# dylanhogan/aggfly

Hardware: AMD Instinct MI355X
Metric: grid-cell-timesteps/s (fused transform+weighted reduce) (higher is better)
Workload: dtype f64

## Files before the change

### aggfly_amd/csrc/afhip_api.hip

```cpp
#include <hip/hip_runtime.h>

#include <algorithm>
#include <cmath>
#include <cstdio>
#include <cstdlib>
#include <cstring>
#include <mutex>
#include <string>
#include <vector>

#include "../../include/aggfly_hip.h"
#include "afhip_kernels.h"
#include "afhip_panel_kernels.h"
#include "afhip_lz4_kernels.h"
#include "afhip_zstd_kernels.h"
#include "afhip_inflate_kernels.h"
#include "afhip_planner.h"
#include "afhip_variants.h"
#include "afhip_sine_p2_table.h"

using namespace afhip;

namespace {

// ... 887 lines not shown
        fa.hb_shift = pl->wg == 64 ? 6 : (pl->wg == 128 ? 7 : 8);
        for (int i = 0; i < MAX_THR; ++i) fa.hb_bin_of_slot[i] = pl->hb_bin_of_slot[i];
        for (int k = 0; k <= pl->hb_n; ++k) {
            const double t = pl->hb_edge[k];
            const float f = (float)t;
            fa.hb_edge[k] = t;
            fa.hb_dn[k] = (double)f > t ? std::nextafterf(f, -INFINITY) : f;
            fa.hb_up[k] = (double)f < t ? std::nextafterf(f, INFINITY) : f;
        }
        fa.hb_w = pl->hb_w; fa.hb_lo0 = pl->hb_lo0; fa.hb_gl = pl->hb_gl; fa.hb_gh = pl->hb_gh;
        fa.hb_wf = (float)pl->hb_w; fa.hb_lo0f = (float)pl->hb_lo0; fa.hb_glf = (float)pl->hb_gl; fa.hb_ghf = (float)pl->hb_gh;
        fa.hb_c0b = pl->hb_c0b; fa.hb_c0bf = (float)pl->hb_c0b;
    }
    HIP_TRY(hipLaunchKernel(fn, grid, dim3((unsigned)pl->wg), args, lds, st));
    return AFHIP_OK;
}

static int launch_combine(afhip_plan* pl, const double* partial, double* cells, double* panel, hipStream_t st) {
    const int64_t C = pl->desc.n_cells, P = pl->desc.P;
    if (P == 0) return AFHIP_OK;
    CombineArgs ca{};
    ca.partial = partial; ca.slot_ptr = pl->d_slot_ptr.p; ca.outer_bounds = pl->d_ob.p;
    ca.cells_out = cells; ca.panel = panel; ca.C = C; ca.P = P; ca.K = pl->K;
    ca.pk = pl->packed ? pl->pk : PackFmt{};
    for (int j = 0; j < pl->K; ++j) {
        ca.outer[j] = pl->cols[(size_t)j].outer;
        ca.round_final[j] = (pl->cols[(size_t)j].rounding & AFHIP_ROUND_FINAL) ? 1 : 0;
    }
    if (P >= 4 && panel) {
        dim3 grid((unsigned)((C + CT_CELLS - 1) / CT_CELLS), (unsigned)((P + CT_PER - 1) / CT_PER));
        if (grid.y > 65535) return fail(AFHIP_E_UNSUPPORTED, "more than 524,280 output periods in one call");
        hipLaunchKernelGGL(k_combine_slots_tiled, grid, dim3(WG), 0, st, ca);
    } else {
        dim3 grid((unsigned)((C + WG - 1) / WG), (unsigned)std::min<int64_t>(P, 65535));
        hipLaunchKernelGGL(k_combine_slots, grid, dim3(WG), 0, st, ca);
    }
    HIP_TRY(hipGetLastError());
    return AFHIP_OK;
}

static int launch_spmm_slots(afhip_plan* pl, const afhip_csr* csr, const double* partial, hipStream_t st,
                             double* num_dev, double* den_dev, double* res_dev, bool* divided) {
    const int64_t P = pl->desc.P, K = pl->K, Q = (K + 1) * P;
    if (csr->nseg * P == 0) return AFHIP_OK;
    SlotSpmmArgs sa{};
    sa.seg_ptr = csr->seg_ptr.p; sa.dst = csr->seg_dst.p; sa.cols = csr->cols.p; sa.w = csr->w.p;
    sa.partial = partial; sa.slot_ptr = pl->d_slot_ptr.p; sa.outer_bounds = pl->d_ob.p; sa.out = pl->sums;
    sa.nseg = csr->nseg; sa.P = P; sa.C = pl->desc.n_cells; sa.K = (int32_t)K;
    sa.p_major = pl->slot_spmm_order >= 0 ? pl->slot_spmm_order : (P >= 8 ? 1 : 0);
    *divided = csr->n_split == 0 && csr->nseg == csr->R;
    if (*divided) { sa.num = num_dev; sa.den = den_dev; sa.res = res_dev; sa.R = csr->R; }
    for (int j = 0; j < pl->K; ++j) {
        sa.outer[j] = pl->cols[(size_t)j].outer;
        sa.round_final[j] = (pl->cols[(size_t)j].rounding & AFHIP_ROUND_FINAL) ? 1 : 0;
    }
    const int64_t mean_len = csr->nnz / std::max<int64_t>(csr->nseg, 1);
    int sub = mean_len > 32 ? 64 : (mean_len > 16 ? 32 : (mean_len > 8 ? 16 : 8));
    if (pl->slot_spmm_sub) sub = pl->slot_spmm_sub;
    const int64_t pairs = csr->nseg * P;
    const int64_t blocks = (pairs * sub + WG - 1) / WG;
    if (blocks > INT32_MAX) return fail(AFHIP_E_UNSUPPORTED, "plan_run: %lld (segment, period) pairs in one call", (long long)pairs);
#define AFHIP_SLOTS_SUB(KB)                                                                                                   \
    switch (sub) {                                                                                                            \
        case 8: hipLaunchKernelGGL((k_csr_spmm_slots<KB, 8>), dim3((unsigned)blocks), dim3(WG), 0, st, sa); break;            \
        case 16: hipLaunchKernelGGL((k_csr_spmm_slots<KB, 16>), dim3((unsigned)blocks), dim3(WG), 0, st, sa); break;          \
        case 32: hipLaunchKernelGGL((k_csr_spmm_slots<KB, 32>), dim3((unsigned)blocks), dim3(WG), 0, st, sa); break;          \
        default: hipLaunchKernelGGL((k_csr_spmm_slots<KB, 64>), dim3((unsigned)blocks), dim3(WG), 0, st, sa); break;          \
    }
    if (K <= 2) { AFHIP_SLOTS_SUB(2) }
    else if (K <= 4) { AFHIP_SLOTS_SUB(4) }
    else if (K <= 8) { AFHIP_SLOTS_SUB(8) }
    else { AFHIP_SLOTS_SUB(16) }
#undef AFHIP_SLOTS_SUB
    HIP_TRY(hipGetLastError());
    if (csr->n_split) {
        const int64_t n = csr->n_split * Q;
        hipLaunchKernelGGL(k_csr_combine_segments, dim3((unsigned)((n + WG - 1) / WG)), dim3(WG), 0, st, pl->sums, csr->split_row.p,
                           csr->split_ptr.p, csr->R, Q, csr->n_split);
        HIP_TRY(hipGetLastError());
    }
    return AFHIP_OK;
}

static int ensure_ws(afhip_plan* pl, int64_t bytes, void* user_ws, int64_t user_bytes, const char* who, char** base) {
    if (user_ws) {
        if (user_bytes < bytes)
            return fail(AFHIP_E_INVALID, "%s: the workspace holds %lld bytes, the run needs %lld (afhip_plan_run_workspace_bytes / afhip_plan_workspace_bytes)",
                        who, (long long)user_bytes, (long long)bytes);
        if ((uintptr_t)user_ws % 256 != 0) return fail(AFHIP_E_INVALID, "%s: the workspace must be 256-byte aligned", who);
        int rc = check_ptr_device(pl, user_ws, who, "the workspace");
        if (rc) return rc;
        *base = (char*)user_ws;
        pl->last_ws = 1;
        return AFHIP_OK;
    }
    if (pl->own_ws_bytes < bytes) {
        if (pl->own_ws) { pl->retired.push_back(pl->own_ws); pl->own_ws = nullptr; pl->own_ws_bytes = 0; }
        HIP_TRY(hipMalloc(&pl->own_ws, (size_t)bytes));
        pl->own_ws_bytes = bytes;
    }
    *base = (char*)pl->own_ws;
    pl->last_ws = 2;
    return AFHIP_OK;
}

extern "C" int afhip_plan_run_temporal(afhip_plan* plan, const void* cube_dev, double* cells_dev,
                                       void* workspace_dev, int64_t workspace_bytes, void* stream) {
    if (!plan || !cube_dev || !cells_dev) return fail(AFHIP_E_INVALID, "plan_run_temporal: NULL argument");
    int rcd = check_cube_device(plan, cube_dev, "plan_run_temporal");
    if (!rcd) rcd = check_ptr_device(plan, cells_dev, "plan_run_temporal", "the per-cell output");
    if (rcd) return rcd;
    GUARD_DEVICE(plan->device);
    hipStream_t st = (hipStream_t)stream;
    char* base;
    int rc = ensure_ws(plan, plan->ws_partial, workspace_dev, workspace_bytes, "plan_run_temporal", &base);
    if (rc) return rc;
    double* partial = (double*)base;
    if ((rc = launch_temporal(plan, cube_dev, partial, st))) return rc;
    return launch_combine(plan, partial, cells_dev, nullptr, st);
}

extern "C" int afhip_plan_run(afhip_plan* plan, const void* cube_dev, const afhip_csr* csr,
                              double* num_dev, double* den_dev, double* res_dev, double* cells_dev,
                              void* workspace_dev, int64_t workspace_bytes, void* stream, float* kernel_ms) {
    if (!plan || !cube_dev || !csr || !res_dev) return fail(AFHIP_E_INVALID, "plan_run: NULL argument");
    if (csr->n_cells != plan->desc.n_cells)
        return fail(AFHIP_E_INVALID, "plan_run: CSR has %lld cells, plan has %lld", (long long)csr->n_cells, (long long)plan->desc.n_cells);
    if (csr->device != plan->device)
        return fail(AFHIP_E_INVALID, "plan_run: the CSR lives on device %d, the plan on device %d", csr->device, plan->device);
    int rcd = check_cube_device(plan, cube_dev, "plan_run");
    if (!rcd) rcd = check_ptr_device(plan, res_dev, "plan_run", "the result panel");
    if (!rcd && num_dev) rcd = check_ptr_device(plan, num_dev, "plan_run", "the numerator panel");
    if (!rcd && den_dev) rcd = check_ptr_device(plan, den_dev, "plan_run", "the denominator panel");
    if (!rcd && cells_dev) rcd = check_ptr_device(plan, cells_dev, "plan_run", "the per-cell output");
    if (rcd) return rcd;
    GUARD_DEVICE(plan->device);
    hipStream_t st = (hipStream_t)stream;
    const int64_t K = plan->K, P = plan->desc.P, Q = (K + 1) * P;
    char* base;
    int rc = ensure_ws(plan, afhip_plan_run_workspace_bytes(plan, csr), workspace_dev, workspace_bytes, "plan_run", &base);
    if (rc) return rc;
    double* partial = (double*)base;
    double* panel = (double*)(base + plan->ws_partial);
    plan->sums = (double*)(base + plan->ws_partial + plan->ws_panel);
    if (kernel_ms) {
        for (auto& e : plan->ev) if (!e) HIP_TRY(hipEventCreate(&e));
        HIP_TRY(hipEventRecord(plan->ev[0], st));
    }
    const bool exact = plan->desc.exact_order != 0 || spmm_serial_env();
    const afhip_csr::RfTab* rf = nullptr;
    if (plan->rf_plan_ok && !exact && !cells_dev && !plan->packed) {
        rf = rf_table(const_cast<afhip_csr*>(csr), plan->variant->vec);
        if (rf && plan->n_slots * (rf->n_runs + rf->n_xcells) * (K + 1) * 8 > plan->ws_partial) rf = nullptr;
    }
    const bool prof = !plan->prof_ev.empty() && (size_t)(2 * plan->prof_count + 1) < plan->prof_ev.size();
    if (prof) HIP_TRY(hipEventRecord(plan->prof_ev[(size_t)(2 * plan->prof_count)], st));
    if ((rc = launch_temporal(plan, cube_dev, partial, st, rf))) return rc;
    if (prof) { HIP_TRY(hipEventRecord(plan->prof_ev[(size_t)(2 * plan->prof_count + 1)], st)); ++plan->prof_count; }
    if (kernel_ms) HIP_TRY(hipEventRecord(plan->ev[1], st));
    plan->last_route = rf ? 1 : 0;
    plan->last_counts_lanes = -1;
    bool divided = false;
    if (rf) {
        const int64_t n = csr->R * P * (K + 1);
        if (n) {
            uint32_t mean_mask = 0;
            for (int j = 0; j < plan->K; ++j) if (plan->cols[(size_t)j].outer == OUT_MEAN) mean_mask |= 1u << j;
            hipLaunchKernelGGL(k_rf_reduce, dim3((unsigned)((n + WG - 1) / WG)), dim3(WG), 0, st, (const double*)partial, rf->reg_ptr.p, rf->reg_runs.p,
                               plan->d_slot_ptr.p, plan->d_ob.p, mean_mask, (const double*)(partial + plan->n_slots * rf->n_runs * (K + 1)), rf->n_xcells,
                               rf->xreg_ptr.p, rf->xcell.p, rf->xw.p, plan->sums, csr->R, P, (int)(K + 1), rf->n_runs,
                               rf_run_major(plan, rf) ? (int64_t)(K + 1) : rf->n_runs * (K + 1), rf_run_major(plan, rf) ? plan->n_slots * (K + 1) : (int64_t)(K + 1),
                               (!rf_run_major(plan, rf) && P >= 8) ? 1 : 0);
            HIP_TRY(hipGetLastError());
        }
    } else if (plan->packed && !cells_dev && plan->n_slots <= P && plan->counts_spmm) {
        const int64_t nv = exact ? csr->R : csr->nseg, nq = nv * P;
        if (nq) {
            divided = (exact || csr->n_split == 0) && nv == csr->R;
            const int64_t nnz_rows = csr->h_indptr.empty() ? 0 : csr->h_indptr.back();
            const double entries = nv > 0 ? (double)nnz_rows / (double)nv : 0.0;
            const int sub_rule = ((double)P < entries) ? (entries < 12.0 ? 8 : 16) : 0;
            const int sub = exact ? 0 : (plan->counts_spmm_sub >= 0 ? plan->counts_spmm_sub : sub_rule);
            plan->last_counts_lanes = (sub == 4 || sub == 8 || sub == 16) ? sub : 1;
            const int64_t* ip = exact ? csr->indptr.p : csr->seg_ptr.p;
            const int32_t* dr = exact ? (const int32_t*)nullptr : csr->seg_dst.p;
            double* o_num = divided ? num_dev : (double*)nullptr; double* o_den = divided ? den_dev : (double*)nullptr; double* o_res = divided ? res_dev : (double*)nullptr;
            if (sub == 4 || sub == 8 || sub == 16) {
                const dim3 gr((unsigned)((nq * sub + WG - 1) / WG)), bl(WG);
                if (sub == 4) hipLaunchKernelGGL((k_csr_spmm_counts_sub<4>), gr, bl, 0, st, ip, dr, csr->cols.p, csr->w.p, (const void*)partial, plan->d_slot_ptr.p, plan->sums, nv, P, (int)K, plan->desc.n_cells, plan->pk, o_num, o_den, o_res);
                else if (sub == 8) hipLaunchKernelGGL((k_csr_spmm_counts_sub<8>), gr, bl, 0, st, ip, dr, csr->cols.p, csr->w.p, (const void*)partial, plan->d_slot_ptr.p, plan->sums, nv, P, (int)K, plan->desc.n_cells, plan->pk, o_num, o_den, o_res);
                else hipLaunchKernelGGL((k_csr_spmm_counts_sub<16>), gr, bl, 0, st, ip, dr, csr->cols.p, csr->w.p, (const void*)partial, plan->d_slot_ptr.p, plan->sums, nv, P, (int)K, plan->desc.n_cells, plan->pk, o_num, o_den, o_res);
            } else
            hipLaunchKernelGGL(k_csr_spmm_counts, dim3((unsigned)((nq + WG - 1) / WG)), dim3(WG), 0, st, ip, dr, csr->cols.p,
                               csr->w.p, (const void*)partial, plan->d_slot_ptr.p, plan->sums, nv, P, (int)K, plan->desc.n_cells, plan->pk,
                               o_num, o_den, o_res);
            HIP_TRY(hipGetLastError());
            if (!exact && csr->n_split) {
                const int64_t n = csr->n_split * Q;
                hipLaunchKernelGGL(k_csr_combine_segments, dim3((unsigned)((n + WG - 1) / WG)), dim3(WG), 0, st, plan->sums, csr->split_row.p,
                                   csr->split_ptr.p, csr->R, Q, csr->n_split);
                HIP_TRY(hipGetLastError());
            }
        }
    } else if (!exact && !cells_dev && !plan->packed && K > 0 && !plan->no_slot_spmm) {
        if ((rc = launch_spmm_slots(plan, csr, partial, st, num_dev, den_dev, res_dev, &divided))) return rc;
    } else {
        if ((rc = launch_combine(plan, partial, cells_dev, panel, st))) return rc;
        if ((rc = launch_spmm(csr, panel, plan->sums, Q, st, exact))) return rc;
    }
    const int64_t n = K > 0 ? csr->R * P : 0;
    if (n && !divided) {
        hipLaunchKernelGGL(k_panel_divide, dim3((unsigned)((n + WG - 1) / WG)), dim3(WG), 0, st, plan->sums, num_dev,
                           den_dev, res_dev, csr->R, P, (int)K);
        HIP_TRY(hipGetLastError());
    }
    if (kernel_ms) {
        HIP_TRY(hipEventRecord(plan->ev[2], st));
        HIP_TRY(hipEventSynchronize(plan->ev[2]));
        HIP_TRY(hipEventElapsedTime(&kernel_ms[0], plan->ev[0], plan->ev[1]));
        HIP_TRY(hipEventElapsedTime(&kernel_ms[1], plan->ev[0], plan->ev[2]));
    }
    return AFHIP_OK;
}

extern "C" int afhip_plan_profile_begin(afhip_plan* plan, int64_t max_launches) {
    if (!plan || max_launches < 0) return fail(AFHIP_E_INVALID, "plan_profile_begin: bad arguments");
    GUARD_DEVICE(plan->device);
    for (auto& e : plan->prof_ev) if (e) (void)hipEventDestroy(e);
    plan->prof_ev.assign((size_t)(2 * max_launches), nullptr);
    for (auto& e : plan->prof_ev) HIP_TRY(hipEventCreate(&e));
    plan->prof_count = 0;
    return AFHIP_OK;
}

extern "C" int64_t afhip_plan_profile_end(afhip_plan* plan, float* ms_out, int64_t cap) {
    if (!plan) return 0;
    DeviceGuard guard__(plan->device);
    const int64_t n = plan->prof_count;
    for (int64_t i = 0; i < n && i < cap; ++i) {
        if (hipEventSynchronize(plan->prof_ev[(size_t)(2 * i + 1)]) != hipSuccess ||
            hipEventElapsedTime(&ms_out[i], plan->prof_ev[(size_t)(2 * i)], plan->prof_ev[(size_t)(2 * i + 1)]) != hipSuccess) {
            fail(AFHIP_E_HIP, "plan_profile_end: event query failed");
            return -1;
        }
    }
    for (auto& e : plan->prof_ev) if (e) (void)hipEventDestroy(e);
    plan->prof_ev.clear();
    plan->prof_count = 0;
    return n;
}

static int run_group(const void* cube_dev, int dtype, int64_t T, int64_t n_cells, const int64_t* bounds,
                     int64_t G, int code, const double* ddargs, int64_t D, void* out_dev, void* stream) {
    if (!cube_dev || !bounds || !out_dev) return fail(AFHIP_E_INVALID, "group kernel: NULL argument");
    if (G < 0 || D <= 0) return fail(AFHIP_E_INVALID, "group kernel: bad G/D");
    if (dtype != AFHIP_F32 && dtype != AFHIP_F64) return fail(AFHIP_E_INVALID, "group kernel: dtype must be AFHIP_F32 or AFHIP_F64");
    if (G == 0) return AFHIP_OK;
// ... 59 lines not shown
```

### aggfly_amd/csrc/afhip_panel_kernels.h

```cpp
#pragma once
#include "afhip_kernels.h"

namespace afhip {

struct CombineArgs {
    const double* partial;
    const int32_t* slot_ptr;
    const int64_t* outer_bounds;
    double* cells_out;
    double* panel;
    int64_t C, P;
    int32_t K;
    int32_t outer[MAX_COLS];
    int32_t round_final[MAX_COLS];
    PackFmt pk;
};

__device__ __forceinline__ double ld_partial(const double* partial, const PackFmt& pk, int64_t s, int j, int K, int64_t C, int64_t c) {
    if (pk.nw) {
        const uint64_t q = ((const uint64_t*)partial)[(s * C + c) * pk.nw + pk.word[j]];
        const uint32_t u = (uint32_t)(q >> pk.shift[j]) & pk.mask;
        return u == pk.mask ? nan64() : (double)u;
    }
    return partial[(s * K + j) * C + c];
// ... 400 lines not shown
                if (a.outer[k] == OUT_MEAN) x[k] = x[k] / ng;
                if (a.round_final[k]) x[k] = (double)(float)x[k];
                valid = valid && (x[k] == x[k]);
            }
        }
#pragma unroll
        for (int k = 0; k < KB; ++k)
            if (k < K) acc[k] = __dadd_rn(acc[k], __dmul_rn(wj, valid ? x[k] : 0.0));
        acc[KB] = __dadd_rn(acc[KB], __dmul_rn(wj, valid ? 1.0 : 0.0));
    };
    auto merged = [&](int k, int64_t c) -> double {
        double val = a.partial[((int64_t)s0 * K + k) * C + c];
        const int o = a.outer[k];
        for (int s = s0 + 1; s < s1; ++s) {
            const double x = a.partial[((int64_t)s * K + k) * C + c];
            if (o == OUT_MIN) { double t = (x < val) ? x : val; val = (x != x || val != val) ? nan64() : t; }
            else if (o == OUT_MAX) { double t = (x > val) ? x : val; val = (x != x || val != val) ? nan64() : t; }
            else if (o == OUT_FIRST) {  }
            else val += x;
        }
        return val;
    };
    if (s1 != s0) {
        const int64_t j0 = a.seg_ptr[v], j1 = a.seg_ptr[v + 1];
        int64_t j = j0 + sl;
        if (s1 == s0 + 1) {
            const double* base = a.partial + (int64_t)s0 * K * C;
            for (; j + (UNR - 1) * SUB < j1; j += UNR * SUB) {
                double x[UNR][KB], wj[UNR];
#pragma unroll
                for (int u = 0; u < UNR; ++u) {
                    const int64_t c = a.cols[j + u * SUB];
                    wj[u] = a.w[j + u * SUB];
#pragma unroll
                    for (int k = 0; k < KB; ++k) x[u][k] = (k < K) ? base[(int64_t)k * C + c] : 0.0;
                }
#pragma unroll
                for (int u = 0; u < UNR; ++u) finish(x[u], wj[u]);
            }
            for (; j < j1; j += SUB) {
                double x[KB];
                const int64_t c = a.cols[j];
#pragma unroll
                for (int k = 0; k < KB; ++k) x[k] = (k < K) ? base[(int64_t)k * C + c] : 0.0;
                finish(x, a.w[j]);
            }
        } else {
            for (; j < j1; j += SUB) {
                double x[KB];
                const int64_t c = a.cols[j];
#pragma unroll
                for (int k = 0; k < KB; ++k) x[k] = (k < K) ? merged(k, c) : 0.0;
                finish(x, a.w[j]);
            }
        }
    }
#pragma unroll
    for (int m = SUB / 2; m >= 1; m >>= 1) {
#pragma unroll
        for (int k = 0; k <= KB; ++k)
            if (k < K || k == KB) acc[k] = __dadd_rn(acc[k], __shfl_xor(acc[k], m, 64));
    }
    if (sl == 0 && live) {
        if (a.res != nullptr) {
            const int64_t RP = a.R * a.P, rp = (int64_t)a.dst[v] * a.P + p;
            const double de = acc[KB];
            if (a.den) a.den[rp] = de;
#pragma unroll
            for (int k = 0; k < KB; ++k) {
                if (k >= K) continue;
                if (a.num) a.num[(int64_t)k * RP + rp] = acc[k];
                a.res[(int64_t)k * RP + rp] = (de != 0.0) ? acc[k] / de : nan64();
            }
            return;
        }
        double* o = a.out + ((int64_t)a.dst[v] * a.P + p) * (K + 1);
#pragma unroll
        for (int k = 0; k < KB; ++k)
            if (k < K) o[k] = acc[k];
        o[K] = acc[KB];
    }
}

__global__ __launch_bounds__(WG) void k_rf_reduce(const double* __restrict__ rf_out, const int64_t* __restrict__ reg_ptr,
                                                  const int32_t* __restrict__ reg_runs, const int32_t* __restrict__ slot_ptr,
                                                  const int64_t* __restrict__ outer_bounds, uint32_t mean_mask,
                                                  const double* __restrict__ ex, int64_t nx, const int64_t* __restrict__ xreg_ptr,
                                                  const int32_t* __restrict__ xcell, const double* __restrict__ xw,
                                                  double* __restrict__ sums, int64_t R, int64_t P, int K1, int64_t n_runs,
                                                  int64_t slot_stride, int64_t run_stride, int p_major) {
    const int64_t tid = (int64_t)blockIdx.x * WG + threadIdx.x;
    if (tid >= R * P * K1) return;
    const int k = (int)(tid % K1);
    const int64_t rp = tid / K1;
    const int64_t r = p_major ? rp % R : rp / P, p = p_major ? rp / R : rp - r * P;
    const int s0 = slot_ptr[p], s1 = slot_ptr[p + 1];
    double acc = 0.0;
    if (s1 != s0) {
        const double* base = rf_out + (int64_t)s0 * slot_stride + k;
        int64_t q = reg_ptr[r];
        const int64_t q1 = reg_ptr[r + 1];
        for (; q + 8 <= q1; q += 8) {
            double v[8];
#pragma unroll
            for (int u = 0; u < 8; ++u) v[u] = base[(int64_t)reg_runs[q + u] * run_stride];
#pragma unroll
            for (int u = 0; u < 8; ++u) acc = __dadd_rn(acc, v[u]);
        }
        for (; q < q1; ++q) acc = __dadd_rn(acc, base[(int64_t)reg_runs[q] * run_stride]);
        if (nx) {
            const double* xb = ex + (int64_t)s0 * nx * K1 + k;
            for (int64_t x = xreg_ptr[r]; x < xreg_ptr[r + 1]; ++x) acc = __dadd_rn(acc, __dmul_rn(xw[x], xb[(int64_t)xcell[x] * K1]));
        }
        if ((mean_mask >> k) & 1u) acc = acc / (double)(outer_bounds[p + 1] - outer_bounds[p]);
    }
    sums[(r * P + p) * K1 + k] = acc;
}

__global__ __launch_bounds__(WG) void k_csr_combine_segments(double* __restrict__ sums, const int32_t* __restrict__ split_row,
                                                             const int32_t* __restrict__ split_ptr, int64_t R, int64_t Q, int64_t n_split) {
    const int64_t tid = (int64_t)blockIdx.x * WG + threadIdx.x;
    if (tid >= n_split * Q) return;
    const int64_t i = tid / Q, q = tid - i * Q;
    double a = 0.0;
    for (int64_t k = split_ptr[i]; k < split_ptr[i + 1]; ++k) a = __dadd_rn(a, sums[(R + k) * Q + q]);
    sums[(int64_t)split_row[i] * Q + q] = a;
}

__global__ __launch_bounds__(WG) void k_panel_divide(const double* __restrict__ sums, double* __restrict__ num,
                                                     double* __restrict__ den, double* __restrict__ res,
                                                     int64_t R, int64_t P, int K) {
    const int64_t rp = (int64_t)blockIdx.x * WG + threadIdx.x;
    const int64_t RP = R * P;
    if (rp >= RP) return;
    const double* rec = sums + rp * (K + 1);
    double v[MAX_COLS + 1];
#pragma unroll
    for (int k = 0; k <= MAX_COLS; ++k) v[k] = (k <= K) ? rec[k] : 0.0;
    double de = 0.0;
#pragma unroll
    for (int k = 0; k <= MAX_COLS; ++k) if (k == K) de = v[k];
    if (den) den[rp] = de;
#pragma unroll
    for (int k = 0; k < MAX_COLS; ++k) {
        if (k >= K) continue;
        if (num) num[(int64_t)k * RP + rp] = v[k];
        res[(int64_t)k * RP + rp] = (de != 0.0) ? v[k] / de : nan64();
    }
}

__global__ __launch_bounds__(WG) void k_divide_num_den(const double* __restrict__ num, const double* __restrict__ den,
                                                       double* __restrict__ res, int64_t n, int64_t RP) {
    const int64_t i = (int64_t)blockIdx.x * WG + threadIdx.x;
    if (i >= n) return;
    const double de = den[i % RP];
    res[i] = (de != 0.0) ? num[i] / de : nan64();
}

__global__ __launch_bounds__(WG) void k_validity_panel(const double* __restrict__ x, double* __restrict__ panel,
                                                       int64_t C, int64_t nt, int K) {
    const int64_t tid = (int64_t)blockIdx.x * WG + threadIdx.x;
    if (tid >= C * nt) return;
    const int64_t c = tid / nt, t = tid - c * nt;
    const int64_t Q = (int64_t)(K + 1) * nt;
    bool valid = true;
    for (int j = 0; j < K; ++j) { const double v = x[((int64_t)j * C + c) * nt + t]; valid = valid && (v == v); }
    for (int j = 0; j < K; ++j) {
        const double v = x[((int64_t)j * C + c) * nt + t];
        panel[c * Q + t * (K + 1) + j] = valid ? v : 0.0;
    }
    panel[c * Q + t * (K + 1) + K] = valid ? 1.0 : 0.0;
}

__global__ __launch_bounds__(WG) void k_unpack_i16(const int16_t* __restrict__ q, int64_t n, const PackArgs p, float* __restrict__ out) {
    const int64_t e0 = ((int64_t)blockIdx.x * WG + threadIdx.x) * 4;
    if (e0 >= n) return;
    if (e0 + 4 <= n) {
        const RawVec<int16_t, 4> r = *(const RawVec<int16_t, 4>*)(q + e0);
        float f[4];
        unpack_i16<4>(r.v, p, f);
        typedef float f4 __attribute__((ext_vector_type(4)));
        *(f4*)(out + e0) = f4{f[0], f[1], f[2], f[3]};
    } else {
        for (int64_t e = e0; e < n; ++e) {
            const int16_t one[1] = {q[e]};
            float f[1];
            unpack_i16<1>(one, p, f);
            out[e] = f[0];
        }
    }
}

constexpr int TRANSFORM_PER_THREAD = 4;
struct TransformArgs {
    const void* x;
    const void* other;
    void* out;
    int64_t n;
    int32_t x_f32, other_f32, out_f32, tf, iarg, pad;
// ... 79 lines not shown
```

### aggfly_amd/csrc/afhip_planner.cpp

```cpp
#include "afhip_planner.h"

#include <algorithm>
#include <cmath>
#include <cstdarg>
#include <cstdio>
#include <cstdlib>
#include <cstring>
#include <string>

namespace afhip {

namespace {
thread_local std::string g_err;
}

int fail(int code, const char* fmt, ...) {
    char buf[1024];
    va_list ap;
    va_start(ap, fmt);
    vsnprintf(buf, sizeof buf, fmt, ap);
    va_end(ap);
    g_err = buf;
    return code;
}

const char* last_error() { return g_err.c_str(); }

PlanKnobs read_knobs() {
    auto set = [](const char* name) { return getenv(name) != nullptr; };
    PlanKnobs k;
    if (const char* e = getenv("AFHIP_FORCE_WG")) { int w = atoi(e); if (w == 64 || w == 128 || w == 256) k.force_wg = w; }
    if (const char* e = getenv("AFHIP_WGS_PER_CU")) k.wgs_per_cu = std::max(1, atoi(e));
    k.no_period_chunks = set("AFHIP_NO_PERIOD_CHUNKS");
    k.no_round_fill = set("AFHIP_NO_ROUND_FILL");
    k.no_pair_mode = set("AFHIP_NO_PAIR_MODE");
    k.no_quad_mode = set("AFHIP_NO_QUAD_MODE");
    k.no_ragged_mode = set("AFHIP_NO_RAGGED_MODE");
    k.no_region_fused = set("AFHIP_NO_REGION_FUSED");
    k.counts_spmm = !set("AFHIP_NO_COUNTS_SPMM");
    if (const char* e = getenv("AFHIP_COUNTS_SPMM_SUB")) k.counts_spmm_sub = atoi(e);
    if (const char* e = getenv("AFHIP_NO_SLOT_SPMM")) k.no_slot_spmm = atoi(e) != 0;
    if (const char* e = getenv("AFHIP_RF_LAYOUT")) k.rf_layout = (e[0] == 'r') ? 1 : 0;
    if (const char* e = getenv("AFHIP_SLOT_SPMM_ORDER")) k.slot_spmm_order = (e[0] == 'p') ? 1 : 0;
    if (const char* e = getenv("AFHIP_SLOT_SPMM_SUB")) { const int sb = atoi(e); if (sb == 8 || sb == 16 || sb == 32 || sb == 64) k.slot_spmm_sub = sb; }
    return k;
}

static int add_thr_slot(std::vector<ThrSlot>& thr, const double* a3, bool bins) {
    ThrSlot s{};
    s.t0 = a3[0]; s.t1 = a3[1];
    const bool base_is_t0 = (a3[2] == 0.0);
    if (bins) { s.A = 0.0; s.B = 1.0; }
    else if (base_is_t0) { s.A = 1.0; s.B = -a3[0]; }
    else { s.A = -1.0; s.B = a3[1]; }
    s.t0f = (float)a3[0]; if ((double)s.t0f > a3[0]) s.t0f = std::nextafterf(s.t0f, -INFINITY);
    s.t1f = (float)a3[1]; if ((double)s.t1f < a3[1]) s.t1f = std::nextafterf(s.t1f, INFINITY);
    s.nan_poisons = bins ? 0 : 1;
    for (size_t i = 0; i < thr.size(); ++i)
        if (!memcmp(&thr[i], &s, sizeof s)) return (int)i;
    thr.push_back(s);
    return (int)thr.size() - 1;
}

static int lower_columns(PlanLayout* pl) {
    const int K = pl->desc.K;
    int stat = 0;
    pl->thr.clear(); pl->cols.clear();
    pl->has_sine = false;
    for (int j = 0; j < K; ++j) {
        const afhip_column& c = pl->columns[j];
        ColOp co{};
        co.rounding = c.rounding;
        switch (c.inner) {
            case AFHIP_MEAN: co.src = SRC_MEAN; stat = std::max(stat, 1); break;
            case AFHIP_SUM: co.src = SRC_SUM; stat = std::max(stat, 1); break;
            case AFHIP_MIN: co.src = SRC_MIN; stat = std::max(stat, 2); break;
            case AFHIP_MAX: co.src = SRC_MAX; stat = std::max(stat, 2); break;
            case AFHIP_NANMEAN: co.src = SRC_NANMEAN; stat = 3; break;
            case AFHIP_DD: co.src = SRC_THR; co.src_idx = add_thr_slot(pl->thr, c.inner_args, false); break;
            case AFHIP_BINS: co.src = SRC_THR; co.src_idx = add_thr_slot(pl->thr, c.inner_args, true); break;
            case AFHIP_SINE_DD:
                co.src = SRC_SINE; stat = std::max(stat, 2);
                co.s0 = c.inner_args[0]; co.s1 = c.inner_args[1];
                co.s0x2 = 2.0 * co.s0; co.s1x2 = 2.0 * co.s1;
                {
                    auto dn = [](double t) { float f = (float)t; return (double)f > t ? std::nextafterf(f, -INFINITY) : f; };
                    auto up = [](double t) { float f = (float)t; return (double)f < t ? std::nextafterf(f, INFINITY) : f; };
                    co.s0dn = dn(co.s0); co.s0up = up(co.s0); co.s1dn = dn(co.s1); co.s1up = up(co.s1);
                }
                co.swidth = co.s1 - co.s0; co.swidth2 = 2.0 * co.swidth;
                pl->has_sine = true;
                if (c.inner_args[2] != 0.0 && c.inner_args[2] != 1.0)
                    return fail(AFHIP_E_INVALID, "column %d: sine_dd flag must be 0 or 1 (temporal.py:324)", j);
                co.skind = (int)c.inner_args[2];
                break;
            default: return fail(AFHIP_E_INVALID, "column %d: unknown inner reducer %d", j, c.inner);
        }
        switch (c.transform) {
            case AFHIP_TF_NONE: co.tf = TF_NONE; break;
            case AFHIP_TF_POW: {
                const double e = c.transform_arg;
                if (e == std::floor(e) && std::fabs(e) <= 64.0) { co.tf = TF_POWI; co.tf_iarg = (int)e; }
                else { co.tf = TF_POW; co.tf_arg = e; }
                break;
            }
            case AFHIP_TF_HINGE: co.tf = TF_HINGE; co.tf_arg = c.transform_arg; break;
            case AFHIP_TF_INTER: co.tf = TF_INTER; break;
            default: return fail(AFHIP_E_INVALID, "column %d: unknown transform %d", j, c.transform);
        }
        if (co.tf == TF_POW || co.tf == TF_INTER) stat = 3;
        switch (c.outer) {
            case AFHIP_IDENTITY: co.outer = OUT_FIRST; break;
            case AFHIP_SUM: co.outer = OUT_SUM; break;
            case AFHIP_MEAN: co.outer = OUT_MEAN; break;
            case AFHIP_MIN: co.outer = OUT_MIN; break;
            case AFHIP_MAX: co.outer = OUT_MAX; break;
            case AFHIP_DD:
            case AFHIP_BINS:
                co.outer = c.outer == AFHIP_DD ? OUT_DD : OUT_BINS;
                co.o0 = c.outer_args[0]; co.o1 = c.outer_args[1];
                co.obase = (c.outer_args[2] == 0.0) ? c.outer_args[0] : c.outer_args[1];
                break;
            default:
                return fail(AFHIP_E_UNSUPPORTED, "column %d: outer reducer %d is not fused (use the staged path)", j, c.outer);
        }
// ... 491 lines not shown
```

### aggfly_amd/csrc/afhip_planner.h

```cpp
#pragma once
#include <stddef.h>
#include <stdint.h>

#include <vector>

#include "../../include/aggfly_hip.h"
#include "afhip_plan_types.h"
#include "afhip_variants.h"

namespace afhip {

int fail(int code, const char* fmt, ...) __attribute__((format(printf, 2, 3)));
const char* last_error();

struct DeviceFacts {
    int cu_count = 0;
    int (*resident_wgs)(const void* fn, int wg, size_t lds) = nullptr;
};

struct RunKnobs {
    bool counts_spmm = true;
    int counts_spmm_sub = -1;
    bool no_slot_spmm = false;
    int slot_spmm_sub = 0;
    int slot_spmm_order = -1;
    int rf_layout = -1;
};

struct PlanKnobs : RunKnobs {
    int force_wg = 0;
    int wgs_per_cu = 0;
    bool no_period_chunks = false, no_round_fill = false;
    bool no_pair_mode = false, no_quad_mode = false, no_ragged_mode = false;
    bool no_region_fused = false;
};
PlanKnobs read_knobs();

struct HistPartition {
    int hb_n = 0; double hb_c1 = 0, hb_c0 = 0;
    bool hb_arith = false; double hb_w = 0, hb_lo0 = 0, hb_gl = 0, hb_gh = 0, hb_c0b = 0;
    int hb_bin_of_slot[MAX_THR] = {0};
    double hb_edge[MAX_THR + 1] = {0};
};

struct PlanLayout : RunKnobs, HistPartition {
    bool has_sine = false;
    afhip_plan_desc desc{};
    std::vector<int64_t> ib, ob;
    std::vector<afhip_column> columns;
    int stat = 0, nthr = 0, K = 0;
    std::vector<ThrSlot> thr;
    std::vector<ColOp> cols;
    std::vector<ChunkDesc> chunks;
    std::vector<int32_t> emit;
    std::vector<int64_t> gtab;
    std::vector<int32_t> slot_ptr;
    int64_t n_slots = 0;
    const Variant* variant = nullptr;
    const Variant* variant_rf = nullptr;
    bool rf_plan_ok = false;
    int64_t tiles = 0;
    int wg = WG;
    bool packed = false;
    PackFmt pk{};
    int64_t ws_partial = 0, ws_panel = 0;
};

int build_plan(const afhip_plan_desc* desc, const DeviceFacts& dev, PlanLayout* out);

size_t plan_lds_bytes(const PlanLayout* pl);

}
```

Measured before the change: 862.4 billion.

## Fuse region-fused reduce with divide/finish and process all columns per thread

Replaces the per-(region,period,column) k_rf_reduce kernel with k_rf_finish, where each thread handles one (region,period) pair across all K+1 columns. Records are read with 2-wide vector loads, and numerator, denominator and ratio are written directly, so the separate divide/finish pass over the sums buffer is skipped (divided=true). An optional LDS transpose tiles regions by periods so the outputs are written in coalesced order. The trade is more registers per thread and fewer threads when R*P is small.

New measurement: 861.3 billion. Within noise of the previous version (-0.1%).

```diff
diff --git a/aggfly_amd/csrc/afhip_api.hip b/aggfly_amd/csrc/afhip_api.hip
--- a/aggfly_amd/csrc/afhip_api.hip
+++ b/aggfly_amd/csrc/afhip_api.hip
@@ -993,6 +993,43 @@
     return AFHIP_OK;
 }
 
+static int launch_rf_finish(afhip_plan* pl, const afhip_csr* csr, const afhip_csr::RfTab* rf, const double* partial, hipStream_t st,
+                            double* num_dev, double* den_dev, double* res_dev) {
+    const int64_t P = pl->desc.P, K = pl->K, R = csr->R;
+    if (K == 0 || R * P == 0) return AFHIP_OK;
+    const bool run_major = rf_run_major(pl, rf);
+    RfFinishArgs fa{};
+    fa.rf_out = partial; fa.reg_ptr = rf->reg_ptr.p; fa.reg_runs = rf->reg_runs.p;
+    fa.slot_ptr = pl->d_slot_ptr.p; fa.outer_bounds = pl->d_ob.p;
+    fa.ex = partial + pl->n_slots * rf->n_runs * (K + 1); fa.nx = rf->n_xcells;
+    fa.xreg_ptr = rf->xreg_ptr.p; fa.xcell = rf->xcell.p; fa.xw = rf->xw.p;
+    fa.num = num_dev; fa.den = den_dev; fa.res = res_dev;
+    fa.R = R; fa.P = P; fa.K = (int32_t)K;
+    fa.slot_stride = run_major ? (int64_t)(K + 1) : rf->n_runs * (K + 1);
+    fa.run_stride = run_major ? pl->n_slots * (K + 1) : (int64_t)(K + 1);
+    for (int j = 0; j < pl->K; ++j) if (pl->cols[(size_t)j].outer == OUT_MEAN) fa.mean_mask |= 1u << j;
+    int tp = (run_major || P < 8) ? 0 : (P >= 32 ? 16 : 4);
+    if (pl->rf_finish_tp >= 0) tp = pl->rf_finish_tp;
+    const int64_t blocks = tp ? ((R + RF_FINISH_TR - 1) / RF_FINISH_TR) * ((P + tp - 1) / tp) : (R * P + WG - 1) / WG;
+    if (blocks > INT32_MAX) return fail(AFHIP_E_UNSUPPORTED, "plan_run: %lld (region, period) pairs in one call", (long long)(R * P));
+    const dim3 gr((unsigned)blocks);
+#define AFHIP_RF_FINISH(KB)                                                                                   \
+    switch (tp) {                                                                                             \
+        case 4: hipLaunchKernelGGL((k_rf_finish<KB, 4>), gr, dim3(RF_FINISH_TR * 4), 0, st, fa); break;       \
+        case 16: hipLaunchKernelGGL((k_rf_finish<KB, 16>), gr, dim3(RF_FINISH_TR * 16), 0, st, fa); break;    \
+        default: hipLaunchKernelGGL((k_rf_finish<KB, 0>), gr, dim3(WG), 0, st, fa); break;                    \
+    }
+    if (K + 1 <= 2) { AFHIP_RF_FINISH(2) }
+    else if (K + 1 <= 4) { AFHIP_RF_FINISH(4) }
+    else if (K + 1 <= 6) { AFHIP_RF_FINISH(6) }
+    else if (K + 1 <= 8) { AFHIP_RF_FINISH(8) }
+    else if (K + 1 <= 12) { AFHIP_RF_FINISH(12) }
+    else { AFHIP_RF_FINISH(MAX_COLS + 1) }
+#undef AFHIP_RF_FINISH
+    HIP_TRY(hipGetLastError());
+    return AFHIP_OK;
+}
+
 static int ensure_ws(afhip_plan* pl, int64_t bytes, void* user_ws, int64_t user_bytes, const char* who, char** base) {
     if (user_ws) {
         if (user_bytes < bytes)
@@ -1073,17 +1110,8 @@
     plan->last_counts_lanes = -1;
     bool divided = false;
     if (rf) {
-        const int64_t n = csr->R * P * (K + 1);
-        if (n) {
-            uint32_t mean_mask = 0;
-            for (int j = 0; j < plan->K; ++j) if (plan->cols[(size_t)j].outer == OUT_MEAN) mean_mask |= 1u << j;
-            hipLaunchKernelGGL(k_rf_reduce, dim3((unsigned)((n + WG - 1) / WG)), dim3(WG), 0, st, (const double*)partial, rf->reg_ptr.p, rf->reg_runs.p,
-                               plan->d_slot_ptr.p, plan->d_ob.p, mean_mask, (const double*)(partial + plan->n_slots * rf->n_runs * (K + 1)), rf->n_xcells,
-                               rf->xreg_ptr.p, rf->xcell.p, rf->xw.p, plan->sums, csr->R, P, (int)(K + 1), rf->n_runs,
-                               rf_run_major(plan, rf) ? (int64_t)(K + 1) : rf->n_runs * (K + 1), rf_run_major(plan, rf) ? plan->n_slots * (K + 1) : (int64_t)(K + 1),
-                               (!rf_run_major(plan, rf) && P >= 8) ? 1 : 0);
-            HIP_TRY(hipGetLastError());
-        }
+        if ((rc = launch_rf_finish(plan, csr, rf, partial, st, num_dev, den_dev, res_dev))) return rc;
+        divided = true;
     } else if (plan->packed && !cells_dev && plan->n_slots <= P && plan->counts_spmm) {
         const int64_t nv = exact ? csr->R : csr->nseg, nq = nv * P;
         if (nq) {
diff --git a/aggfly_amd/csrc/afhip_panel_kernels.h b/aggfly_amd/csrc/afhip_panel_kernels.h
--- a/aggfly_amd/csrc/afhip_panel_kernels.h
+++ b/aggfly_amd/csrc/afhip_panel_kernels.h
@@ -506,39 +506,129 @@
     }
 }
 
-__global__ __launch_bounds__(WG) void k_rf_reduce(const double* __restrict__ rf_out, const int64_t* __restrict__ reg_ptr,
-                                                  const int32_t* __restrict__ reg_runs, const int32_t* __restrict__ slot_ptr,
-                                                  const int64_t* __restrict__ outer_bounds, uint32_t mean_mask,
-                                                  const double* __restrict__ ex, int64_t nx, const int64_t* __restrict__ xreg_ptr,
-                                                  const int32_t* __restrict__ xcell, const double* __restrict__ xw,
-                                                  double* __restrict__ sums, int64_t R, int64_t P, int K1, int64_t n_runs,
-                                                  int64_t slot_stride, int64_t run_stride, int p_major) {
-    const int64_t tid = (int64_t)blockIdx.x * WG + threadIdx.x;
-    if (tid >= R * P * K1) return;
-    const int k = (int)(tid % K1);
-    const int64_t rp = tid / K1;
-    const int64_t r = p_major ? rp % R : rp / P, p = p_major ? rp / R : rp - r * P;
-    const int s0 = slot_ptr[p], s1 = slot_ptr[p + 1];
-    double acc = 0.0;
-    if (s1 != s0) {
-        const double* base = rf_out + (int64_t)s0 * slot_stride + k;
-        int64_t q = reg_ptr[r];
-        const int64_t q1 = reg_ptr[r + 1];
-        for (; q + 8 <= q1; q += 8) {
-            double v[8];
-#pragma unroll
-            for (int u = 0; u < 8; ++u) v[u] = base[(int64_t)reg_runs[q + u] * run_stride];
-#pragma unroll
-            for (int u = 0; u < 8; ++u) acc = __dadd_rn(acc, v[u]);
-        }
-        for (; q < q1; ++q) acc = __dadd_rn(acc, base[(int64_t)reg_runs[q] * run_stride]);
-        if (nx) {
-            const double* xb = ex + (int64_t)s0 * nx * K1 + k;
-            for (int64_t x = xreg_ptr[r]; x < xreg_ptr[r + 1]; ++x) acc = __dadd_rn(acc, __dmul_rn(xw[x], xb[(int64_t)xcell[x] * K1]));
-        }
-        if ((mean_mask >> k) & 1u) acc = acc / (double)(outer_bounds[p + 1] - outer_bounds[p]);
-    }
-    sums[(r * P + p) * K1 + k] = acc;
+struct RfFinishArgs {
+    const double* rf_out;
+    const int64_t* reg_ptr;
+    const int32_t* reg_runs;
+    const int32_t* slot_ptr;
+    const int64_t* outer_bounds;
+    const double* ex;
+    const int64_t* xreg_ptr;
+    const int32_t* xcell;
+    const double* xw;
+    double *num, *den, *res;
+    int64_t nx, R, P, slot_stride, run_stride;
+    uint32_t mean_mask;
+    int32_t K;
+};
+
+constexpr int RF_FINISH_TR = 16;
+
+template <int K1B, int TP>
+__global__ __launch_bounds__(WG) void k_rf_finish(const RfFinishArgs a) {
+    typedef double d2 __attribute__((ext_vector_type(2)));
+    constexpr int U = K1B > 8 ? 2 : (K1B > 4 ? 4 : 8);
+    const int K = a.K, K1 = K + 1;
+    const bool v2 = (K1 & 1) == 0;
+    int64_t r, p;
+    bool mine;
+    if constexpr (TP == 0) {
+        const int64_t rp = (int64_t)blockIdx.x * WG + threadIdx.x;
+        mine = rp < a.R * a.P;
+        r = mine ? rp / a.P : 0;
+        p = mine ? rp - r * a.P : 0;
+    } else {
+        const int64_t nbr = (a.R + RF_FINISH_TR - 1) / RF_FINISH_TR;
+        const int64_t bp = blockIdx.x / nbr, br = blockIdx.x - bp * nbr;
+        r = br * RF_FINISH_TR + (threadIdx.x % RF_FINISH_TR);
+        p = bp * TP + (threadIdx.x / RF_FINISH_TR);
+        mine = r < a.R && p < a.P;
+        if (!mine) { r = 0; p = 0; }
+    }
+    auto ld_rec = [&](const double* rec, double (&v)[K1B]) {
+        if (v2) {
+#pragma unroll
+            for (int j = 0; j < K1B / 2; ++j)
+                if (2 * j < K1) { const d2 t = ((const d2*)rec)[j]; v[2 * j] = t.x; v[2 * j + 1] = t.y; }
+        } else {
+#pragma unroll
+            for (int k = 0; k < K1B; ++k)
+                if (k < K1) v[k] = rec[k];
+        }
+    };
+    double acc[K1B];
+#pragma unroll
+    for (int k = 0; k < K1B; ++k) acc[k] = 0.0;
+    const int s0 = a.slot_ptr[p], s1 = a.slot_ptr[p + 1];
+    if (mine && s1 != s0) {
+        const double* base = a.rf_out + (int64_t)s0 * a.slot_stride;
+        int64_t q = a.reg_ptr[r];
+        const int64_t q1 = a.reg_ptr[r + 1];
+        for (; q + U <= q1; q += U) {
+            double v[U][K1B];
+#pragma unroll
+            for (int u = 0; u < U; ++u) ld_rec(base + (int64_t)a.reg_runs[q + u] * a.run_stride, v[u]);
+#pragma unroll
+            for (int u = 0; u < U; ++u)
+#pragma unroll
+                for (int k = 0; k < K1B; ++k)
+                    if (k < K1) acc[k] = __dadd_rn(acc[k], v[u][k]);
+        }
+        for (; q < q1; ++q) {
+            double v[K1B];
+            ld_rec(base + (int64_t)a.reg_runs[q] * a.run_stride, v);
+#pragma unroll
+            for (int k = 0; k < K1B; ++k)
+                if (k < K1) acc[k] = __dadd_rn(acc[k], v[k]);
+        }
+        if (a.nx) {
+            const double* xb = a.ex + (int64_t)s0 * a.nx * K1;
+            for (int64_t x = a.xreg_ptr[r]; x < a.xreg_ptr[r + 1]; ++x) {
+                double v[K1B];
+                ld_rec(xb + (int64_t)a.xcell[x] * K1, v);
+                const double w = a.xw[x];
+#pragma unroll
+                for (int k = 0; k < K1B; ++k)
+                    if (k < K1) acc[k] = __dadd_rn(acc[k], __dmul_rn(w, v[k]));
+            }
+        }
+        if (a.mean_mask) {
+            const double n = (double)(a.outer_bounds[p + 1] - a.outer_bounds[p]);
+#pragma unroll
+            for (int k = 0; k < K1B; ++k)
+                if (k < K1 && ((a.mean_mask >> k) & 1u)) acc[k] = acc[k] / n;
+        }
+    }
+    int64_t o = r * a.P + p;
+    if constexpr (TP > 0) {
+        __shared__ double turn[K1B][RF_FINISH_TR * (TP + 1)];
+#pragma unroll
+        for (int k = 0; k < K1B; ++k)
+            if (k < K1) turn[k][(threadIdx.x % RF_FINISH_TR) * (TP + 1) + threadIdx.x / RF_FINISH_TR] = acc[k];
+        __syncthreads();
+        const int rl = threadIdx.x / TP, pl = threadIdx.x % TP;
+#pragma unroll
+        for (int k = 0; k < K1B; ++k)
+            if (k < K1) acc[k] = turn[k][rl * (TP + 1) + pl];
+        const int64_t nbr = (a.R + RF_FINISH_TR - 1) / RF_FINISH_TR;
+        const int64_t bp = blockIdx.x / nbr, br = blockIdx.x - bp * nbr;
+        r = br * RF_FINISH_TR + rl;
+        p = bp * TP + pl;
+        mine = r < a.R && p < a.P;
+        o = r * a.P + p;
+    }
+    if (!mine) return;
+    const int64_t RP = a.R * a.P;
+    double de = 0.0;
+#pragma unroll
+    for (int k = 0; k < K1B; ++k) if (k == K) de = acc[k];
+    if (a.den) a.den[o] = de;
+#pragma unroll
+    for (int k = 0; k < K1B - 1; ++k) {
+        if (k >= K) continue;
+        if (a.num) a.num[(int64_t)k * RP + o] = acc[k];
+        a.res[(int64_t)k * RP + o] = (de != 0.0) ? acc[k] / de : nan64();
+    }
 }
 
 __global__ __launch_bounds__(WG) void k_csr_combine_segments(double* __restrict__ sums, const int32_t* __restrict__ split_row,
diff --git a/aggfly_amd/csrc/afhip_planner.cpp b/aggfly_amd/csrc/afhip_planner.cpp
--- a/aggfly_amd/csrc/afhip_planner.cpp
+++ b/aggfly_amd/csrc/afhip_planner.cpp
@@ -41,6 +41,7 @@
     if (const char* e = getenv("AFHIP_COUNTS_SPMM_SUB")) k.counts_spmm_sub = atoi(e);
     if (const char* e = getenv("AFHIP_NO_SLOT_SPMM")) k.no_slot_spmm = atoi(e) != 0;
     if (const char* e = getenv("AFHIP_RF_LAYOUT")) k.rf_layout = (e[0] == 'r') ? 1 : 0;
+    if (const char* e = getenv("AFHIP_RF_FINISH_TP")) { const int tp = atoi(e); if (tp == 0 || tp == 4 || tp == 16) k.rf_finish_tp = tp; }
     if (const char* e = getenv("AFHIP_SLOT_SPMM_ORDER")) k.slot_spmm_order = (e[0] == 'p') ? 1 : 0;
     if (const char* e = getenv("AFHIP_SLOT_SPMM_SUB")) { const int sb = atoi(e); if (sb == 8 || sb == 16 || sb == 32 || sb == 64) k.slot_spmm_sub = sb; }
     return k;
diff --git a/aggfly_amd/csrc/afhip_planner.h b/aggfly_amd/csrc/afhip_planner.h
--- a/aggfly_amd/csrc/afhip_planner.h
+++ b/aggfly_amd/csrc/afhip_planner.h
@@ -25,6 +25,7 @@
     int slot_spmm_sub = 0;
     int slot_spmm_order = -1;
     int rf_layout = -1;
+    int rf_finish_tp = -1;
 };
 
 struct PlanKnobs : RunKnobs {
```
